# nasa/PROTEUS

Hardware: AMD Instinct MI355X
Metric: Mpixels/sec DSWx classify (3660^2 7-band HLS tiles) (higher is better)
Workload: dtype int16+f64

## Files before the change

### proteus_amd/build.py

```python
import contextlib
import fcntl
import hashlib
import os
import shutil
import subprocess
import sys

PKG = os.path.dirname(os.path.abspath(__file__))
ROOT = os.path.dirname(PKG)
CSRC = os.path.join(PKG, 'csrc')
LAB = os.path.join(ROOT, 'tools', 'lab', 'csrc')
SOURCES = [os.path.join(CSRC, n) for n in ('dswx_hip.hip', 'dswx_classify_lut.hip', 'dswx_cover.hip',
                                           'dswx_layers.hip', 'dswx_host_path.hip', 'dswx_batch.hip', 'dswx_writer.hip',
                                           'dswx_checksum.hip', 'dswx_compare.hip', 'dswx_histogram.hip', 'dswx_crosstab.hip',
                                           'dswx_stack.hip', 'dswx_grid.hip', 'dswx_label.hip', 'dswx_body_table.hip',
                                           'dswx_distance.hip', 'dswx_outline.hip', 'dswx_burn.hip', 'dswx_mosaic.hip', 'dswx_warp.hip',
                                           'dswx_resample.hip')]
HEADERS = [os.path.join(CSRC, n) for n in ('dswx_device.h', 'dswx_host.h', 'dswx_tables.h', 'dswx_vmm.h',
                                           'dswx_hist_bin.h', 'dswx_stack_rule.h', 'dswx_grid_rule.h',
                                           'dswx_label_rule.h', 'dswx_body_rule.h', 'dswx_distance_rule.h',
                                           'dswx_outline_rule.h', 'dswx_burn_rule.h', 'dswx_batch_select.h',
                                           'dswx_mesh_rule.h', 'dswx_resample_rule.h')]
LAB_SOURCES = [os.path.join(LAB, n) for n in ('dswx_lab.hip', 'dswx_probes.hip')]
LAB_HEADERS = [os.path.join(LAB, 'dswx_lab.h')]
INCLUDE = os.path.join(ROOT, 'include')
PUBLIC_HEADER = os.path.join(INCLUDE, 'dswx_hip.h')
LIB_DIR = os.path.join(PKG, '_lib')
LIB_PATH = os.path.join(LIB_DIR, 'libdswx_hip.so')
LAB_PATH = os.path.join(LIB_DIR, 'libdswx_lab.so')

HIPCC_FLAGS = ['--offload-arch=gfx950', '-O3', '-std=c++17', '-fPIC', '-shared',
               '-ffp-contract=off', '-Wall', '-Wno-unused-function']
HOT_KERNEL_SOURCES = [os.path.join(CSRC, n) for n in ('dswx_classify_lut.hip', 'dswx_tables.h', 'dswx_device.h')]


def find_hipcc():
    for cand in (shutil.which('hipcc'), '/opt/rocm/bin/hipcc'):
        if cand and os.path.exists(cand):
            return cand
    return None


def _digest(paths, extra=b''):
    h = hashlib.sha256(extra)
    for path in paths:
        h.update(os.path.basename(path).encode() + b'\0')
        with open(path, 'rb') as f:
            h.update(f.read())
        h.update(b'\0')
    return h.hexdigest()


def _stamp(lib):
    return lib + '.srchash'


def _stale(lib, deps, extra=b''):
    if not os.path.exists(lib) or not os.path.exists(_stamp(lib)):
        return True
    try:
        with open(_stamp(lib)) as f:
            return f.read().strip() != _digest(deps, extra)
    except OSError:
        return True


def _product_deps():
    return SOURCES + HEADERS + [PUBLIC_HEADER]


def _lab_deps():
    return LAB_SOURCES + LAB_HEADERS + HEADERS + [PUBLIC_HEADER]


def _flags_tag():
    return ' '.join(HIPCC_FLAGS).encode()


def is_stale():
    return _stale(LIB_PATH, _product_deps(), _flags_tag())


def _product_stamp():
    try:
        with open(_stamp(LIB_PATH)) as f:
            return f.read().strip().encode()
    except OSError:
        return b'missing'


def lab_is_stale():
    return _stale(LAB_PATH, _lab_deps(), _flags_tag() + _product_stamp())


def hot_kernel_hash():
    h = hashlib.sha256()
    for path in HOT_KERNEL_SOURCES:
        with open(path, 'rb') as f:
            h.update(f.read())
    return h.hexdigest()[:16]


def _run(cmd, verbose):
    if verbose:
        print(' '.join(cmd), file=sys.stderr)
    res = subprocess.run(cmd, capture_output=True, text=True)
    if res.returncode != 0:
        raise RuntimeError(f'{os.path.basename(cmd[0])} failed:\n' + res.stdout + res.stderr)


@contextlib.contextmanager
def _build_lock():
    os.makedirs(LIB_DIR, exist_ok=True)
    try:
        f = open(os.path.join(LIB_DIR, '.build.lock'), 'a')
    except OSError:
        yield
        return
    with f:
        fcntl.flock(f, fcntl.LOCK_EX)
        try:
            yield
        finally:
            fcntl.flock(f, fcntl.LOCK_UN)


def _write_stamp(lib, digest):
    tmp = f'{_stamp(lib)}.{os.getpid()}.tmp'
    with open(tmp, 'w') as f:
        f.write(digest + '\n')
    os.replace(tmp, _stamp(lib))


def _need_hipcc(lib):
    hipcc = find_hipcc()
    if hipcc is None:
        raise RuntimeError(f'hipcc not found and {os.path.relpath(lib, ROOT)} is '
                           + ('not the build of these sources (content digest differs)' if os.path.exists(lib) else 'missing')
                           + ' (need ROCm for the gfx950 build)')
    return hipcc


def build(force=False, verbose=False):
    if not force and not is_stale():
        return LIB_PATH
    with _build_lock():
        if not force and not is_stale():
            return LIB_PATH
        hipcc = _need_hipcc(LIB_PATH)
        tmp = f'{LIB_PATH}.{os.getpid()}.tmp'
        digest = _digest(_product_deps(), _flags_tag())
        _run([hipcc] + HIPCC_FLAGS + ['-I', INCLUDE, '-I', CSRC] + SOURCES + ['-o', tmp], verbose)
        if os.path.exists(_stamp(LIB_PATH)):
            os.remove(_stamp(LIB_PATH))
        os.replace(tmp, LIB_PATH)
        _write_stamp(LIB_PATH, digest)
    return LIB_PATH


def build_lab(force=False, verbose=False):
    build(force=False, verbose=verbose)
    if not force and not lab_is_stale():
        return LAB_PATH
    with _build_lock():
        if not force and not lab_is_stale():
            return LAB_PATH
        hipcc = _need_hipcc(LAB_PATH)
        tmp = f'{LAB_PATH}.{os.getpid()}.tmp'
        digest = _digest(_lab_deps(), _flags_tag() + _product_stamp())
        _run([hipcc] + HIPCC_FLAGS + ['-I', INCLUDE, '-I', CSRC, '-I', LAB] + LAB_SOURCES +
             ['-L', LIB_DIR, '-ldswx_hip', '-Wl,-rpath,$ORIGIN', '-o', tmp], verbose)
        if os.path.exists(_stamp(LAB_PATH)):
            os.remove(_stamp(LAB_PATH))
        os.replace(tmp, LAB_PATH)
        _write_stamp(LAB_PATH, digest)
# ... 74 lines not shown
```

### proteus_amd/csrc/dswx_host.h

```cpp
#pragma once

#include <hip/hip_runtime.h>
#include <cstddef>
#include <cstdint>
#include <cstring>
#include <mutex>
#include <string>

#include "dswx_device.h"
#include "dswx_mesh_rule.h"

struct dswx_workspace {
    void* p = nullptr;
    size_t bytes = 0;
};

struct dswx_ctx {
    int device = -1;
    hipStream_t stream = nullptr;
    enum { WS_STAGE, WS_PARTIALS, WS_FOLD, WS_COVER, WS_UNTILE, WS_COUNT };
    dswx_workspace ws[WS_COUNT];
    bool fold_clean = false;
    hipStream_t ws_last = nullptr;
    bool ws_used = false;
    hipEvent_t ws_event = nullptr;
    void* tables = nullptr;
    bool tables_valid = false;
    hipStream_t tables_stream = nullptr;
    alignas(8) unsigned char tables_params[1024] = {};
    hipStream_t h2d_stream = nullptr, d2h_stream = nullptr;
    hipEvent_t pipe_in[3] = {nullptr, nullptr, nullptr}, pipe_k[3] = {nullptr, nullptr, nullptr},
               pipe_out[3] = {nullptr, nullptr, nullptr};
    int64_t* pipe_counters = nullptr;
    size_t pipe_counters_cap = 0;
    int cover_kernel = 8;
    int host_pipeline = 2;
    int host_chunks = 8;
    int shadow_kernel = 0;
    int shadow_grid_pad = 1;
    std::string last_kernel;
    int tune_lut_wps = 0;
    int tune_lut_interleave = -1;
    int tune_wps = 6;
    int tune_fold = 1;
    int place_force_candidate = -1;
    int fused_variant = -1;
};

int dswx_ws_enter(dswx_ctx* ctx, hipStream_t s);
int dswx_ws_leave(dswx_ctx* ctx, hipStream_t s);

int dswx_fail(int code, const char* fmt, ...);
int dswx_make_dev_params(const dswx_params_t* p, DevParams* d);

#define HIP_TRY(expr)                                                                              \
    do {                                                                                           \
        hipError_t e__ = (expr);                                                                   \
        if (e__ != hipSuccess)                                                                     \
            return dswx_fail(DSWX_ERR_HIP, "%s failed: %s (%s:%d)", #expr, hipGetErrorString(e__), \
                             __FILE__, __LINE__);                                                  \
    } while (0)

std::mutex& dswx_va_mutex();
template <typename T>
static inline hipError_t dswx_locked_malloc(T** p, size_t n) {
    std::lock_guard<std::mutex> lock(dswx_va_mutex());
    return hipMalloc(reinterpret_cast<void**>(p), n);
}

static inline hipStream_t dswx_stream_of(const dswx_ctx* ctx, void* stream) { return stream ? (hipStream_t)stream : ctx->stream; }

struct dswx_call_scratch {
    hipStream_t s;
    void* p[4] = {nullptr, nullptr, nullptr, nullptr};
    int n = 0;
    bool queued = false;
    explicit dswx_call_scratch(hipStream_t stream) : s(stream) {}
    dswx_call_scratch(const dswx_call_scratch&) = delete;
    template <typename T>
    hipError_t take(T** out, size_t bytes) {
        if (n == 4) return hipErrorOutOfMemory;
        const hipError_t e = dswx_locked_malloc(out, bytes);
        if (e == hipSuccess) { p[n++] = *out; queued = true; }
        return e;
    }
    hipError_t sync() {
        const hipError_t e = hipStreamSynchronize(s);
        if (e == hipSuccess) queued = false;
        return e;
    }
    ~dswx_call_scratch() {
        if (queued) (void)hipStreamSynchronize(s);
        for (int i = 0; i < n; ++i) (void)hipFree(p[i]);
    }
};

static inline bool aligned_to(const void* p, size_t a) { return (reinterpret_cast<uintptr_t>(p) & (a - 1)) == 0; }

int dswx_ws_reserve(dswx_workspace& w, size_t need, hipStream_t s, bool whole_device = false);

struct dswx_plane_desc {
    const char* name;
    bool input;
    unsigned char bytes;
    signed char batch;
    unsigned short offset;
    signed char kind;
};
#define DSWX_BAND_(k) {"band[" #k "]", true, 2, DSWX_PLANE_BAND0 + k, offsetof(dswx_planes_in_t, band) + k * sizeof(void*), DSWX_CMP_I16}
#define DSWX_IN_(f, idx) {#f, true, 1, idx, offsetof(dswx_planes_in_t, f), DSWX_CMP_U8}
#define DSWX_OUT_(f, bytes, idx) \
    {#f, false, bytes, idx, offsetof(dswx_planes_out_t, f), bytes == 1 ? DSWX_CMP_U8 : bytes == 2 ? DSWX_CMP_U16 : DSWX_CMP_F64}
constexpr dswx_plane_desc DSWX_PLANES[] = {
    DSWX_BAND_(0), DSWX_BAND_(1), DSWX_BAND_(2), DSWX_BAND_(3), DSWX_BAND_(4), DSWX_BAND_(5),
    DSWX_IN_(fmask, DSWX_PLANE_FMASK), DSWX_IN_(land, DSWX_PLANE_LAND), DSWX_IN_(shad, DSWX_PLANE_SHAD),
    DSWX_IN_(ocean, DSWX_PLANE_OCEAN),
    DSWX_OUT_(diag, 2, DSWX_PLANE_DIAG), DSWX_OUT_(wtr1, 1, DSWX_PLANE_WTR1),
    DSWX_OUT_(wtr1_aerosol, 1, DSWX_PLANE_WTR1_AEROSOL), DSWX_OUT_(wtr2, 1, DSWX_PLANE_WTR2),
    DSWX_OUT_(wtr, 1, DSWX_PLANE_WTR), DSWX_OUT_(bwtr, 1, DSWX_PLANE_BWTR), DSWX_OUT_(conf, 1, DSWX_PLANE_CONF),
    DSWX_OUT_(cloud, 1, DSWX_PLANE_CLOUD), DSWX_OUT_(browse, 1, DSWX_PLANE_BROWSE),
    DSWX_OUT_(mndwi, 8, -1), DSWX_OUT_(ndvi, 8, -1), DSWX_OUT_(awesh, 8, -1),
};
#undef DSWX_BAND_
#undef DSWX_IN_
#undef DSWX_OUT_
constexpr int DSWX_N_PLANES = sizeof DSWX_PLANES / sizeof DSWX_PLANES[0];

constexpr bool dswx_planes_in_abi_order() {
    constexpr int n_in = sizeof(dswx_planes_in_t) / sizeof(void*);
    for (int i = 0; i < DSWX_N_PLANES; ++i) {
        const dswx_plane_desc& d = DSWX_PLANES[i];
        if (d.input != (i < n_in) || d.offset != (d.input ? i : i - n_in) * sizeof(void*)) return false;
        if (d.batch != (i < DSWX_PLANE_COUNTERS ? i : -1)) return false;
    }
    return true;
}
static_assert(sizeof(dswx_planes_in_t) + sizeof(dswx_planes_out_t) == DSWX_N_PLANES * sizeof(void*) &&
              dswx_planes_in_abi_order(), "DSWX_PLANES does not match dswx_planes_in_t / dswx_planes_out_t");

static inline char* dswx_plane_get(const dswx_plane_desc& d, const dswx_planes_in_t* in, const dswx_planes_out_t* out) {
    const char* s = d.input ? reinterpret_cast<const char*>(in) : reinterpret_cast<const char*>(out);
    char* p = nullptr;
    if (s) std::memcpy(&p, s + d.offset, sizeof p);
    return p;
}
static inline void dswx_plane_set(const dswx_plane_desc& d, dswx_planes_in_t* in, dswx_planes_out_t* out, const void* p) {
    char* s = d.input ? reinterpret_cast<char*>(in) : reinterpret_cast<char*>(out);
    if (s) std::memcpy(s + d.offset, &p, sizeof p);
}

constexpr int DSWX_FOLD_MAX_TILES = 16;

int dswx_lut_fold_group_log2(bool extras);
void dswx_lut_geometry(const dswx_ctx* ctx, long long groups, bool extras, int lead_max, int* threads, long long* gx);
int dswx_lut_launch(dswx_ctx* ctx, const KArgs& args, bool masks, dim3 grid, dim3 block, hipStream_t stream,
                    char* info, size_t info_len);

struct dswx_checksum_plane {
    const void* base;
    uint64_t tile_bytes;
    uint64_t stride_bytes;
};
int dswx_checksum_launch(dswx_ctx* ctx, const dswx_checksum_plane* planes, int n_planes, int64_t n_tiles, uint64_t* out,
                         hipStream_t s);

struct dswx_compare_pair {
    const void* a;
    const void* b;
    int kind;
    uint64_t n_elems;
    uint64_t a_stride_elems, b_stride_elems;
};
int dswx_compare_elem_bytes(int kind);
int dswx_compare_check_tol(double atol, double rtol);
int dswx_compare_launch(dswx_ctx* ctx, const dswx_compare_pair* pairs, int n_pairs, int64_t n_tiles, double atol, double rtol,
                        int equal_nan, dswx_compare_t* out, hipStream_t s);

struct dswx_histogram_plane {
    const void* base;
    int kind;
    int lo, shift;
    uint64_t n_elems;
    uint64_t stride_elems;
};
int dswx_histogram_elem_bytes(int kind);
int dswx_histogram_check_kind(int kind, int shift);
int dswx_histogram_launch(dswx_ctx* ctx, const dswx_histogram_plane* planes, int n_planes, int64_t n_tiles, uint64_t* out,
                          hipStream_t s);

struct dswx_crosstab_item {
    const void* a;
// ... 91 lines not shown
```

### proteus_amd/csrc/dswx_layers.hip

```cpp
#include <hip/hip_runtime.h>
#include <cmath>
#include <cstring>
#include <limits>

#include "dswx_host.h"

__global__ __launch_bounds__(256) void dswx_interpret_v1(const long long* __restrict__ diag,
                                                         uint8_t* __restrict__ out, long long n) {
    const long long i = (long long)blockIdx.x * 256 + threadIdx.x;
    if (i >= n) return;
    const long long d = diag[i];
    uint32_t cls = 255u;
    if (d >= 0 && d < 32) {
        const uint32_t k = (uint32_t)d;
        cls = ((CLS_B0 >> k) & 1u) | (((CLS_B1 >> k) & 1u) << 1) | (((CLS_B2 >> k) & 1u) << 2);
    }
    out[i] = (uint8_t)cls;
}

struct ShadowArgs {
    const float* dem;
    uint8_t* shadow;
    long long height, width, margin;
    long long out_stride;
    float spacing_x, neg_abs_spacing_y;
    double sun[3];
    double sin_az, cos_az;
    double inc_q_min, slope_arg_max;
    int by_first, by_step;
};

template <bool F32>
__device__ __forceinline__ bool shadow_px_exact(const ShadowArgs& a, float dx, float sx, float dy, float sy) {
    const float gx = dx * sx, gy = dy * sy;
    const float n0 = -gx / a.spacing_x;
    const float n1 = -gy / a.neg_abs_spacing_y;
    const float norm = sqrtf(n0 * n0 + n1 * n1 + 1.0f);
    bool low_inc, backslope;
    if (F32) {
        const float qf = (n0 * (float)a.sun[0] + n1 * (float)a.sun[1] + (float)a.sun[2]) / norm;
        const float tf = n0 * (float)a.sin_az + n1 * (float)a.cos_az;
        low_inc = (qf >= (float)a.inc_q_min) & (qf <= 1.0f);
        backslope = tf <= (float)a.slope_arg_max;
    } else {
        const double dot = (double)n0 * a.sun[0] + (double)n1 * a.sun[1] + a.sun[2];
        const double q = dot / (double)norm;
        const double t = (double)n0 * a.sin_az + (double)n1 * a.cos_az;
        low_inc = (q >= a.inc_q_min) & (q <= 1.0);
        backslope = t <= a.slope_arg_max;
    }
    return low_inc | !backslope;
}

template <bool F32>
__global__ __launch_bounds__(256) void dswx_shadow_v2(const ShadowArgs a) {
    const int W = (int)a.width, H = (int)a.height, margin = (int)a.margin;
    const int ow = W - 2 * margin, oh = H - 2 * margin;
    const int ox = blockIdx.x * 64 + (threadIdx.x & 63), oy = blockIdx.y * 4 + (threadIdx.x >> 6);
    if (ox >= ow || oy >= oh) return;
    const int x = ox + margin, y = oy + margin;
    const float* __restrict__ d = a.dem + (size_t)blockIdx.z * (size_t)H * (size_t)W;
    const int c = y * W + x;
    const bool x_in = (x > 0) & (x < W - 1), y_in = (y > 0) & (y < H - 1);
    const float dx = d[x < W - 1 ? c + 1 : c] - d[x > 0 ? c - 1 : c];
    const float dy = d[y < H - 1 ? c + W : c] - d[y > 0 ? c - W : c];
    const bool v = shadow_px_exact<F32>(a, dx, x_in ? 0.5f : 1.0f, dy, y_in ? 0.5f : 1.0f);
    a.shadow[(size_t)blockIdx.z * (size_t)a.out_stride + (size_t)(oy * ow + ox)] = v ? 1 : 0;
}

struct ShadowFilter {
    float inv_x, inv_y;
    float s0, s1, s2, sin_az, cos_az;
    float q_c, q_h_in, q_h_out;
    float t_c;
    float e_rel, e_abs;
    float et_rel;
    int t_tiny;
};

typedef float f32x2 __attribute__((ext_vector_type(2)));
typedef f32x2 __attribute__((aligned(4))) f32x2_u;
typedef uint32_t __attribute__((aligned(1))) u32_u;

template <bool F32, bool TINY>
__device__ __forceinline__ uint32_t shadow_quad(const ShadowArgs& a, const ShadowFilter& f, f32x2 c0, f32x2 c1, f32x2 c2,
                                                f32x2 c3, f32x2 u0, f32x2 u1, f32x2 b0, f32x2 b1) {
    const f32x2 dx[2] = {f32x2{c1.y, c2.x} - f32x2{c0.y, c1.x}, f32x2{c2.y, c3.x} - f32x2{c1.y, c2.x}};
    const f32x2 dy[2] = {b0 - u0, b1 - u1};
    uint32_t out = 0, unsure = 0;
#pragma unroll
    for (int p = 0; p < 2; ++p) {
        const f32x2 n0 = dx[p] * f.inv_x, n1 = dy[p] * f.inv_y;
        const f32x2 S = __builtin_elementwise_fma(n0, n0, __builtin_elementwise_fma(n1, n1, f32x2{1.0f, 1.0f}));
        const f32x2 dot = __builtin_elementwise_fma(n0, f32x2{f.s0, f.s0},
                                                    __builtin_elementwise_fma(n1, f32x2{f.s1, f.s1}, f32x2{f.s2, f.s2}));
        const f32x2 v = __builtin_elementwise_fma(n0, f32x2{f.sin_az, f.sin_az},
                                                  __builtin_elementwise_fma(n1, f32x2{f.cos_az, f.cos_az}, f32x2{-f.t_c, -f.t_c}));
        const f32x2 r = {__builtin_amdgcn_rsqf(S.x), __builtin_amdgcn_rsqf(S.y)};
        const f32x2 u = __builtin_elementwise_fma(dot, r, f32x2{-f.q_c, -f.q_c});
        f32x2 e = __builtin_elementwise_fma(S * r, f32x2{f.e_rel, f.e_rel}, f32x2{f.e_abs, f.e_abs});
        if (TINY) {
#pragma unroll
            for (int h = 0; h < 2; ++h)
                e[h] = f.et_rel * __builtin_fmaf(__builtin_fabsf(n0[h]), __builtin_fabsf(f.sin_az),
                                                 __builtin_fabsf(n1[h]) * __builtin_fabsf(f.cos_az)) +
                       __builtin_fminf((__builtin_fabsf(dx[p][h]) + __builtin_fabsf(dy[p][h])) * 0x1p100f, 0x1p-120f);
        }
#pragma unroll
        for (int h = 0; h < 2; ++h) {
            const bool sane = S[h] < 0x1p60f;
            const float au = __builtin_fabsf(u[h]), av = __builtin_fabsf(v[h]);
            const bool inc_yes = au <= f.q_h_in, inc_no = au > f.q_h_out;
            const bool back_known = av > e[h], back_no = back_known & (v[h] > 0.0f);
            const bool back_yes = TINY ? ((back_known & (v[h] < 0.0f)) | ((e[h] == 0.0f) & (v[h] <= 0.0f)))
                                           : (back_known & !(v[h] > 0.0f));
            const bool one = sane & (inc_yes | back_no);
            const bool zero = sane & inc_no & back_yes;
            const int k = 2 * p + h;
            out |= (one ? 1u : 0u) << (8 * k);
            unsure |= ((one | zero) ? 0u : 1u) << k;
        }
    }
    if (unsure) {
        const float cx[6] = {c0.y, c1.x, c1.y, c2.x, c2.y, c3.x};
        const float up[4] = {u0.x, u0.y, u1.x, u1.y}, dn[4] = {b0.x, b0.y, b1.x, b1.y};
#pragma unroll 1
        for (int k = 0; k < 4; ++k) {
            if (!((unsure >> k) & 1u)) continue;
            const bool v = shadow_px_exact<F32>(a, cx[k + 2] - cx[k], 0.5f, dn[k] - up[k], 0.5f);
            out = (out & ~(0xffu << (8 * k))) | ((v ? 1u : 0u) << (8 * k));
        }
    }
    return out;
}

constexpr int SHADOW_ROWS = 2, SHADOW_WAVES = 4;

template <bool F32, bool TINY>
__global__ __launch_bounds__(64 * SHADOW_WAVES) void dswx_shadow_v3(const ShadowArgs a, const ShadowFilter f) {
    const int W = (int)a.width, H = (int)a.height, margin = (int)a.margin;
    const int ow = W - 2 * margin, oh = H - 2 * margin;
    const int oq = blockIdx.x * 64 + (threadIdx.x & 63);
    const int oy0 = ((a.by_first + (int)blockIdx.y * a.by_step) * SHADOW_WAVES + (threadIdx.x >> 6)) * SHADOW_ROWS;
    if (4 * oq >= ow || oy0 >= oh) return;
    const int ox = 4 * oq + 4 <= ow ? 4 * oq : ow - 4;
    const float* __restrict__ col = a.dem + (size_t)blockIdx.z * (size_t)H * (size_t)W + (size_t)(ox + margin);
    uint8_t* __restrict__ dst = a.shadow + (size_t)blockIdx.z * (size_t)a.out_stride + (size_t)ox;
    struct Row { f32x2 v[4]; };
    auto load_row = [&](int y) {
        const float* r = col + (size_t)(y < H ? y : H - 1) * (size_t)W;
        return Row{{*reinterpret_cast<const f32x2_u*>(r - 2), *reinterpret_cast<const f32x2_u*>(r),
                    *reinterpret_cast<const f32x2_u*>(r + 2), *reinterpret_cast<const f32x2_u*>(r + 4)}};
    };
    const int y0 = oy0 + margin;
    Row up = load_row(y0 - 1), ce = load_row(y0), dn = load_row(y0 + 1), nx = SHADOW_ROWS > 1 ? load_row(y0 + 2) : dn;
#pragma unroll
    for (int i = 0; i < SHADOW_ROWS; ++i) {
        const Row nn = i + 3 <= SHADOW_ROWS ? load_row(y0 + i + 3) : nx;
        if (oy0 + i < oh) {
            const uint32_t out = shadow_quad<F32, TINY>(a, f, ce.v[0], ce.v[1], ce.v[2], ce.v[3], up.v[1], up.v[2], dn.v[1], dn.v[2]);
            __builtin_nontemporal_store(out, reinterpret_cast<u32_u*>(dst + (size_t)(oy0 + i) * (size_t)ow));
        }
        up = ce;
        ce = dn;
        dn = nx;
        nx = nn;
    }
}

struct LandArgs {
    const uint8_t* wc3;
    const uint8_t* cgls;
    uint8_t* land;
    long long height, width;
    long long out_stride;
    uint32_t forest_bits[8];
    int thr_tree, thr_low, thr_high, thr_water;
    int low_class, high_class;
};

__device__ __forceinline__ int land_class(const LandArgs& a, int water, int urban, int tree, bool is_forest) {
    if (!is_forest) tree = 0;
    int v = 255;
    if (tree >= a.thr_tree) v = 201;
    if (urban >= a.thr_low) v = a.low_class;
    if (urban >= a.thr_high) v = a.high_class;
    if (water >= a.thr_water) v = 200;
    return v;
}

constexpr int LAND_ROWS = 1;

__global__ __launch_bounds__(256) void dswx_landcover_v3(const LandArgs a) {
    __shared__ uint16_t s_code[256];
    __shared__ uint8_t s_forest[256];
    {
        const int v = threadIdx.x;
        s_code[v] = (uint16_t)((((v == 80) | (v == 90) | (v == 95)) ? 1 : 0) | (v == 50 ? 16 : 0) | (v == 10 ? 256 : 0));
        s_forest[v] = (uint8_t)((a.forest_bits[v >> 5] >> (v & 31)) & 1u);
    }
    __syncthreads();
    const unsigned quads_per_row = (unsigned)(a.width >> 2);
    const unsigned q = blockIdx.x * 256u + threadIdx.x;
    const unsigned yq = q / quads_per_row;
    const long long xq = q - yq * quads_per_row, y0 = yq;
    if (y0 >= a.height) return;
    const long long W3 = 3 * a.width, tile = blockIdx.z;
    const uint8_t* wc = a.wc3 + tile * 9 * a.height * a.width;
    uint32_t w[LAND_ROWS][3][3], cg[LAND_ROWS];
#pragma unroll
    for (int r = 0; r < LAND_ROWS; ++r) {
        const long long y = y0 + r < a.height ? y0 + r : a.height - 1;
#pragma unroll
        for (int i = 0; i < 3; ++i) {
            const uint32_t* row = reinterpret_cast<const uint32_t*>(wc + (3 * y + i) * W3 + 12 * xq);
#pragma unroll
            for (int k = 0; k < 3; ++k) w[r][i][k] = row[k];
        }
        cg[r] = __builtin_nontemporal_load(reinterpret_cast<const uint32_t*>(a.cgls + tile * a.height * a.width + y * a.width + 4 * xq));
    }
#pragma unroll
    for (int r = 0; r < LAND_ROWS; ++r) {
        if (y0 + r >= a.height) break;
        uint32_t cnt[4] = {0u, 0u, 0u, 0u};
#pragma unroll
        for (int i = 0; i < 3; ++i) {
#pragma unroll
            for (int j = 0; j < 12; ++j) cnt[j / 3] += s_code[(w[r][i][j >> 2] >> (8 * (j & 3))) & 0xffu];
        }
        uint32_t out = 0;
#pragma unroll
        for (int k = 0; k < 4; ++k)
            out |= (uint32_t)land_class(a, cnt[k] & 15u, (cnt[k] >> 4) & 15u, cnt[k] >> 8,
                                        s_forest[(cg[r] >> (8 * k)) & 0xffu] != 0) << (8 * k);
        __builtin_nontemporal_store(out, reinterpret_cast<uint32_t*>(a.land + tile * a.out_stride + (y0 + r) * a.width + 4 * xq));
    }
}

__global__ __launch_bounds__(256) void dswx_landcover_v1(const LandArgs a) {
    const long long x = (long long)blockIdx.x * 64 + (threadIdx.x & 63);
    const long long y = (long long)blockIdx.y * 4 + (threadIdx.x >> 6);
    if (x >= a.width || y >= a.height) return;
    int water = 0, urban = 0, tree = 0;
    const long long W3 = 3 * a.width;
    const long long tile = blockIdx.z;
#pragma unroll
    for (int i = 0; i < 3; ++i) {
        const uint8_t* row = a.wc3 + tile * 9 * a.height * a.width + (3 * y + i) * W3 + 3 * x;
#pragma unroll
        for (int j = 0; j < 3; ++j) {
            const int v = row[j];
            water += (v == 80) | (v == 90) | (v == 95);
            urban += v == 50;
            tree += v == 10;
        }
    }
    const long long o = tile * a.height * a.width + y * a.width + x;
    const int c = a.cgls[o];
    a.land[tile * a.out_stride + y * a.width + x] = (uint8_t)land_class(a, water, urban, tree, ((a.forest_bits[c >> 5] >> (c & 31)) & 1u) != 0);
}

__device__ __forceinline__ unsigned long long mix64(unsigned long long x) {
    x ^= x >> 30; x *= 0xBF58476D1CE4E5B9ull;
    x ^= x >> 27; x *= 0x94D049BB133111EBull;
    return x ^ (x >> 31);
}
__device__ __forceinline__ long long fieldu(unsigned long long h, int shift, int bits) {
    return (long long)((h >> shift) & ((1ull << bits) - 1ull));
}

__global__ __launch_bounds__(256) void dswx_synth_v1(dswx_planes_in_t in, unsigned long long seed,
                                                      long long tile0, long long n_pixels, int width,
                                                      long long tile_stride) {
    const long long px = (long long)blockIdx.x * 256 + threadIdx.x;
    if (px >= n_pixels) return;
    const long long t = blockIdx.y;
    const unsigned long long tile = (unsigned long long)(tile0 + t);
    const long long off = t * tile_stride + px;
    const unsigned long long K0 = 0x9E3779B97F4A7C15ull, K1 = 0xD1B54A32D192ED03ull;
    const unsigned long long h0 = mix64(seed * K0 + tile * K1 + (unsigned long long)px);
    const unsigned long long h1 = mix64(h0 + K0);
    const unsigned long long h2 = mix64(h1 + K0);
    const int cuts[5] = {14418, 26214, 42598, 55705, 64225};
    const int mean[5][6] = {{350, 450, 350, 250, 150, 100},
                            {500, 700, 600, 1300, 800, 500},
                            {300, 600, 400, 3500, 1800, 900},
                            {900, 1200, 1500, 2200, 2800, 2300},
                            {6000, 6200, 6400, 6600, 3000, 2500}};
    const int amps[5] = {300, 600, 600, 800, 2500};
    const int draw = (int)fieldu(h0, 0, 16);
    int stype = 0;
#pragma unroll
    for (int k = 0; k < 5; ++k) stype += draw >= cuts[k] ? 1 : 0;
    const bool is_fill = stype == 5;
    const int st = stype < 4 ? stype : 4;
    const long long amp = amps[st];
    const bool clip_evt = fieldu(h0, 16, 7) == 0;
    const int clip_band = (int)((fieldu(h0, 23, 3) * 6) >> 3);
    const long long clip_val = -fieldu(h0, 26, 8);
    const bool wrap_evt = fieldu(h0, 34, 10) == 0;
#pragma unroll
    for (int b = 0; b < 6; ++b) {
        const long long noise = fieldu(h1, 10 * b, 10);
        long long v = mean[st][b] + ((noise * 2 * amp) >> 10) - amp;
        if (wrap_evt && (b == 1 || b == 4)) v += 19000;
        if (clip_evt && clip_band == b) v = clip_val;
        if (is_fill) v = -9999;
        const_cast<int16_t*>(in.band[b])[off] = (int16_t)v;
    }
    const long long aerosol = fieldu(h2, 0, 2);
    const long long water = fieldu(h2, 2, 5) < 10, snow = fieldu(h2, 7, 5) < 2,
                    shadow = fieldu(h2, 12, 5) < 3, adjacent = fieldu(h2, 17, 5) < 3,
                    cloud = fieldu(h2, 22, 5) < 4, cirrus = fieldu(h2, 27, 5) < 1;
    long long fm = (aerosol << 6) | (water << 5) | (snow << 4) | (shadow << 3) | (adjacent << 2) |
                   (cloud << 1) | cirrus;
    if (is_fill) fm = 255;
    const_cast<uint8_t*>(in.fmask)[off] = (uint8_t)fm;
    if (in.land) {
        const int classes[8] = {200, 201, 21, 121, 50, 150, 99, 100};
        const int cls = classes[fieldu(h2, 40, 3)];
        const_cast<uint8_t*>(in.land)[off] = (uint8_t)(fieldu(h2, 32, 8) < 179 ? 255 : cls);
    }
    if (in.shad) const_cast<uint8_t*>(in.shad)[off] = (uint8_t)(fieldu(h2, 43, 5) >= 3 ? 1 : 0);
    if (in.ocean) {
        const unsigned long long row_band = (unsigned long long)(px / width) >> 5;
        const unsigned long long hb = mix64(seed * K1 + tile * K0 + row_band + 0x5851F42D4C957F2Dull);
        const_cast<uint8_t*>(in.ocean)[off] = (uint8_t)(fieldu(hb, 0, 8) >= 13 ? 1 : 0);
    }
}

extern "C" {

#define ENTRY_TRY(entry, expr)                                                                                      \
    do {                                                                                                            \
        if (hipError_t e__ = (expr)) return dswx_fail(DSWX_ERR_HIP, entry ": %s", hipGetErrorString(e__));          \
    } while (0)

int dswx_interpret_layer_host(dswx_ctx_t* ctx, const int64_t* diag_decimal, int64_t n, uint8_t* out) {
    if (!ctx || (n > 0 && (!diag_decimal || !out))) return dswx_fail(DSWX_ERR_ARG, "NULL argument");
    if (n < 0) return dswx_fail(DSWX_ERR_ARG, "negative size");
    if (n == 0) return DSWX_OK;
    HIP_TRY(hipSetDevice(ctx->device));
    dswx_call_scratch scratch(ctx->stream);
    long long* d_in = nullptr; uint8_t* d_out = nullptr;
    ENTRY_TRY("dswx_interpret_layer_host", scratch.take(&d_in, (size_t)n * 8));
    ENTRY_TRY("dswx_interpret_layer_host", scratch.take(&d_out, (size_t)n));
    ENTRY_TRY("dswx_interpret_layer_host", hipMemcpyAsync(d_in, diag_decimal, (size_t)n * 8, hipMemcpyHostToDevice, scratch.s));
    hipLaunchKernelGGL(dswx_interpret_v1, dim3((unsigned)((n + 255) / 256)), dim3(256), 0, scratch.s, d_in, d_out, (long long)n);
    ENTRY_TRY("dswx_interpret_layer_host", hipGetLastError());
    ENTRY_TRY("dswx_interpret_layer_host", hipMemcpyAsync(out, d_out, (size_t)n, hipMemcpyDeviceToHost, scratch.s));
    ENTRY_TRY("dswx_interpret_layer_host", scratch.sync());
    return DSWX_OK;
}

static int64_t ord_of(double d) {
    int64_t i;
    std::memcpy(&i, &d, 8);
    return i >= 0 ? i : -(i & 0x7fffffffffffffffLL);
}
static double dbl_of(int64_t k) {
    int64_t i = k >= 0 ? k : (int64_t)(0x8000000000000000ULL | (uint64_t)(-k));
    double d;
    std::memcpy(&d, &i, 8);
    return d;
}
static const double kRad2Deg = 180.0 / 3.141592653589793238462643383279502884;

int dswx_shadow_thresholds(double min_slope_angle, double max_sun_local_inc_angle, double* slope_arg_max,
                           double* inc_q_min) {
    if (!slope_arg_max || !inc_q_min) return dswx_fail(DSWX_ERR_ARG, "NULL argument");
    if (std::isnan(min_slope_angle) || std::isnan(max_sun_local_inc_angle))
        return dswx_fail(DSWX_ERR_ARG, "shadow angle threshold is NaN");
    auto inc_ok = [&](double q) { return std::acos(q) * kRad2Deg <= max_sun_local_inc_angle; };
    if (!inc_ok(1.0)) *inc_q_min = 2.0;
    else if (inc_ok(-1.0)) *inc_q_min = -1.0;
    else {
        int64_t lo = ord_of(-1.0), hi = ord_of(1.0);
        while ((uint64_t)hi - (uint64_t)lo > 1) {
            const int64_t mid = lo + (int64_t)(((uint64_t)hi - (uint64_t)lo) / 2);
            if (inc_ok(dbl_of(mid))) hi = mid; else lo = mid;
        }
        *inc_q_min = dbl_of(hi);
    }
    auto slope_ok = [&](double t) { return std::atan(t) * kRad2Deg <= min_slope_angle; };
    const double inf = std::numeric_limits<double>::infinity();
    if (slope_ok(inf)) *slope_arg_max = inf;
    else if (!slope_ok(-inf)) *slope_arg_max = -inf;
    else {
        int64_t lo = ord_of(-inf), hi = ord_of(inf);
// ... 68 lines not shown
        f->t_c = t_max > 0 ? std::numeric_limits<float>::infinity() : -std::numeric_limits<float>::infinity();
        f->e_abs = 0.0f;
    } else {
        f->t_c = (float)t_max;
        f->e_abs = f->t_tiny ? 0.0f : float_up(std::fabs((double)f->t_c - t_max) + std::fabs(t_max) * 0x1p-20 + 1e-40);
    }
}

static int shadow_launch(dswx_ctx_t* ctx, const ShadowArgs& req, int64_t n_tiles, bool f32, hipStream_t s) {
    if (n_tiles == 0) return DSWX_OK;
    HIP_TRY(hipSetDevice(ctx->device));
    ShadowArgs a = req;
    const long long margin = a.margin, ow = a.width - 2 * margin, oh = a.height - 2 * margin;
    const bool quads = margin >= 2 && ow >= 4 && aligned_to(a.dem, 4) && ctx->shadow_kernel != 2;
    if (quads) {
        ShadowFilter f;
        shadow_filter(a, f32, &f);
        const long long pad = ctx->shadow_grid_pad > 0 ? ctx->shadow_grid_pad : 1;
        const long long gx = (((ow + 3) / 4 + 63) / 64 + pad - 1) / pad * pad;
        const unsigned block_rows = (unsigned)((oh + SHADOW_WAVES * SHADOW_ROWS - 1) / (SHADOW_WAVES * SHADOW_ROWS));
        const dim3 block(64 * SHADOW_WAVES);
        const int passes = ctx->shadow_kernel == 3 ? 2 : 1;
        for (int pass = 0; pass < passes; ++pass) {
            a.by_first = pass; a.by_step = passes;
            const unsigned gy = (block_rows - (unsigned)pass + (unsigned)passes - 1) / (unsigned)passes;
            if (gy == 0) continue;
            const dim3 grid((unsigned)gx, gy, (unsigned)n_tiles);
            if (f32 && f.t_tiny) hipLaunchKernelGGL((dswx_shadow_v3<true, true>), grid, block, 0, s, a, f);
            else if (f32) hipLaunchKernelGGL((dswx_shadow_v3<true, false>), grid, block, 0, s, a, f);
            else if (f.t_tiny) hipLaunchKernelGGL((dswx_shadow_v3<false, true>), grid, block, 0, s, a, f);
            else hipLaunchKernelGGL((dswx_shadow_v3<false, false>), grid, block, 0, s, a, f);
        }
    } else {
        dim3 grid((unsigned)((ow + 63) / 64), (unsigned)((oh + 3) / 4), (unsigned)n_tiles), block(256);
        if (f32) hipLaunchKernelGGL(dswx_shadow_v2<true>, grid, block, 0, s, a);
        else hipLaunchKernelGGL(dswx_shadow_v2<false>, grid, block, 0, s, a);
    }
    HIP_TRY(hipGetLastError());
    return DSWX_OK;
}

static int shadow_host_run(dswx_ctx_t* ctx, ShadowArgs a, bool f32) {
    const float* dem = a.dem; uint8_t* shadow = a.shadow;
    HIP_TRY(hipSetDevice(ctx->device));
    const size_t in_bytes = (size_t)a.height * (size_t)a.width * 4;
    const size_t out_px = (size_t)(a.height - 2 * a.margin) * (size_t)(a.width - 2 * a.margin);
    dswx_call_scratch scratch(ctx->stream);
    float* d_dem = nullptr; uint8_t* d_out = nullptr;
    ENTRY_TRY("dswx_shadow_layer_host", scratch.take(&d_dem, in_bytes));
    ENTRY_TRY("dswx_shadow_layer_host", scratch.take(&d_out, out_px));
    ENTRY_TRY("dswx_shadow_layer_host", hipMemcpyAsync(d_dem, dem, in_bytes, hipMemcpyHostToDevice, scratch.s));
    a.dem = d_dem; a.shadow = d_out;
    if (int rc = shadow_launch(ctx, a, 1, f32, scratch.s)) return rc;
    ENTRY_TRY("dswx_shadow_layer_host", hipMemcpyAsync(shadow, d_out, out_px, hipMemcpyDeviceToHost, scratch.s));
    ENTRY_TRY("dswx_shadow_layer_host", scratch.sync());
    return DSWX_OK;
}

int dswx_shadow_layer_device_q(dswx_ctx_t* ctx, const float* dem, int64_t n_tiles, int64_t height, int64_t width,
                               int64_t margin, const double sun_vector[3], double sin_azimuth,
                               double cos_azimuth, double slope_arg_max, double inc_q_min,
                               double pixel_spacing_x, double pixel_spacing_y, uint8_t* shadow, void* stream) {
    ShadowArgs a;
    if (int rc = shadow_check(&a, ctx, dem, n_tiles, height, width, margin, sun_vector, sin_azimuth, cos_azimuth, slope_arg_max,
                              inc_q_min, pixel_spacing_x, pixel_spacing_y, shadow, 0)) return rc;
    return shadow_launch(ctx, a, n_tiles, false, dswx_stream_of(ctx, stream));
}

int dswx_shadow_layer_device_q32(dswx_ctx_t* ctx, const float* dem, int64_t n_tiles, int64_t height, int64_t width,
                                 int64_t margin, const double sun_vector[3], double sin_azimuth,
                                 double cos_azimuth, float slope_arg_max, float inc_q_min,
                                 double pixel_spacing_x, double pixel_spacing_y, uint8_t* shadow, void* stream) {
    ShadowArgs a;
    if (int rc = shadow_check(&a, ctx, dem, n_tiles, height, width, margin, sun_vector, sin_azimuth, cos_azimuth,
                              (double)slope_arg_max, (double)inc_q_min, pixel_spacing_x, pixel_spacing_y, shadow, 0)) return rc;
    return shadow_launch(ctx, a, n_tiles, true, dswx_stream_of(ctx, stream));
}

int dswx_shadow_layer_device(dswx_ctx_t* ctx, const float* dem, int64_t n_tiles, int64_t height, int64_t width,
                             int64_t margin, const double sun_vector[3], double sin_azimuth,
                             double cos_azimuth, double min_slope_angle, double max_sun_local_inc_angle,
                             double pixel_spacing_x, double pixel_spacing_y, uint8_t* shadow, void* stream) {
    double slope_arg_max, inc_q_min;
    if (int rc = dswx_shadow_thresholds(min_slope_angle, max_sun_local_inc_angle, &slope_arg_max, &inc_q_min)) return rc;
    ShadowArgs a;
    if (int rc = shadow_check(&a, ctx, dem, n_tiles, height, width, margin, sun_vector, sin_azimuth, cos_azimuth, slope_arg_max,
                              inc_q_min, pixel_spacing_x, pixel_spacing_y, shadow, 0)) return rc;
    return shadow_launch(ctx, a, n_tiles, false, dswx_stream_of(ctx, stream));
}

int dswx_shadow_layer_batch(dswx_ctx_t* ctx, const float* dem, int64_t n_tiles, int64_t height, int64_t width,
                            int64_t margin, const double sun_vector[3], double sin_azimuth, double cos_azimuth,
                            double slope_arg_max, double inc_q_min, int32_t float32_arithmetic, double pixel_spacing_x,
                            double pixel_spacing_y, uint8_t* shadow, int64_t shadow_tile_stride, void* stream) {
    ShadowArgs a;
    if (int rc = shadow_check(&a, ctx, dem, n_tiles, height, width, margin, sun_vector, sin_azimuth, cos_azimuth, slope_arg_max,
                              inc_q_min, pixel_spacing_x, pixel_spacing_y, shadow, shadow_tile_stride)) return rc;
    return shadow_launch(ctx, a, n_tiles, float32_arithmetic != 0, dswx_stream_of(ctx, stream));
}

int dswx_shadow_layer_host_q(dswx_ctx_t* ctx, const float* dem, int64_t height, int64_t width, int64_t margin,
                             const double sun_vector[3], double sin_azimuth, double cos_azimuth,
                             double slope_arg_max, double inc_q_min, double pixel_spacing_x,
                             double pixel_spacing_y, uint8_t* shadow) {
    ShadowArgs a;
    if (int rc = shadow_check(&a, ctx, dem, 1, height, width, margin, sun_vector, sin_azimuth, cos_azimuth, slope_arg_max,
                              inc_q_min, pixel_spacing_x, pixel_spacing_y, shadow, 0)) return rc;
    return shadow_host_run(ctx, a, false);
}

int dswx_shadow_layer_host_q32(dswx_ctx_t* ctx, const float* dem, int64_t height, int64_t width, int64_t margin,
                               const double sun_vector[3], double sin_azimuth, double cos_azimuth,
                               float slope_arg_max, float inc_q_min, double pixel_spacing_x,
                               double pixel_spacing_y, uint8_t* shadow) {
    ShadowArgs a;
    if (int rc = shadow_check(&a, ctx, dem, 1, height, width, margin, sun_vector, sin_azimuth, cos_azimuth,
                              (double)slope_arg_max, (double)inc_q_min, pixel_spacing_x, pixel_spacing_y, shadow, 0)) return rc;
    return shadow_host_run(ctx, a, true);
}

int dswx_shadow_layer_host(dswx_ctx_t* ctx, const float* dem, int64_t height, int64_t width, int64_t margin,
                           const double sun_vector[3], double sin_azimuth, double cos_azimuth,
                           double min_slope_angle, double max_sun_local_inc_angle, double pixel_spacing_x,
                           double pixel_spacing_y, uint8_t* shadow) {
    double slope_arg_max, inc_q_min;
    if (int rc = dswx_shadow_thresholds(min_slope_angle, max_sun_local_inc_angle, &slope_arg_max, &inc_q_min)) return rc;
    ShadowArgs a;
    if (int rc = shadow_check(&a, ctx, dem, 1, height, width, margin, sun_vector, sin_azimuth, cos_azimuth, slope_arg_max,
                              inc_q_min, pixel_spacing_x, pixel_spacing_y, shadow, 0)) return rc;
    return shadow_host_run(ctx, a, false);
}

static int land_check(LandArgs* a, dswx_ctx_t* ctx, const uint8_t* worldcover_up3, const uint8_t* copernicus, int64_t n_tiles,
                      int64_t height, int64_t width, const int32_t* forest_classes, int32_t n_forest_classes,
                      const int32_t thresholds[4], int32_t year_offset, uint8_t* land, int64_t land_tile_stride) {
    if (!ctx || !worldcover_up3 || !copernicus || !land) return dswx_fail(DSWX_ERR_ARG, "NULL argument");
    if (land_tile_stride != 0 && land_tile_stride < height * width)
        return dswx_fail(DSWX_ERR_ARG, "land_tile_stride smaller than the raster");
    if (n_tiles < 0 || n_tiles > 65535) return dswx_fail(DSWX_ERR_ARG, "n_tiles out of range");
    if (!thresholds) return dswx_fail(DSWX_ERR_ARG, "NULL argument");
    if (height < 0 || width < 0 || n_forest_classes < 0 || (n_forest_classes > 0 && !forest_classes))
        return dswx_fail(DSWX_ERR_ARG, "bad size");
    std::memset(a, 0, sizeof *a);
    for (int i = 0; i < n_forest_classes; ++i) {
        const int c = forest_classes[i];
        if (c >= 0 && c <= 255) a->forest_bits[c >> 5] |= 1u << (c & 31);
    }
    a->thr_tree = thresholds[0]; a->thr_low = thresholds[1]; a->thr_high = thresholds[2]; a->thr_water = thresholds[3];
    a->low_class = (int)(uint8_t)(0u + (uint32_t)year_offset);
    a->high_class = (int)(uint8_t)(100u + (uint32_t)year_offset);
    a->height = height; a->width = width;
    a->wc3 = worldcover_up3; a->cgls = copernicus; a->land = land;
    a->out_stride = land_tile_stride ? land_tile_stride : height * width;
    return DSWX_OK;
}

static int land_launch(dswx_ctx_t* ctx, const LandArgs& a, int64_t n_tiles, hipStream_t s) {
    const long long height = a.height, width = a.width;
    if (n_tiles == 0 || height == 0 || width == 0) return DSWX_OK;
    HIP_TRY(hipSetDevice(ctx->device));
    const bool quad = width % 4 == 0 && aligned_to(a.wc3, 4) && aligned_to(a.cgls, 4) && aligned_to(a.land, 4) &&
                      a.out_stride % 4 == 0;
    if (quad) {
        static_assert(LAND_ROWS == 1, "the flat quad numbering assumes one row per thread");
        const long long quads = (width / 4) * height;
        if (quads > 0xffffffffLL - 256) return dswx_fail(DSWX_ERR_ARG, "raster too large for one launch");
        dim3 grid((unsigned)((quads + 255) / 256), 1, (unsigned)n_tiles), block(256);
        hipLaunchKernelGGL(dswx_landcover_v3, grid, block, 0, s, a);
    } else {
        dim3 grid((unsigned)((width + 63) / 64), (unsigned)((height + 3) / 4), (unsigned)n_tiles), block(256);
        if (grid.y > 65535) return dswx_fail(DSWX_ERR_ARG, "raster too tall for one launch");
        hipLaunchKernelGGL(dswx_landcover_v1, grid, block, 0, s, a);
    }
    HIP_TRY(hipGetLastError());
    return DSWX_OK;
}

int dswx_landcover_mask_device(dswx_ctx_t* ctx, const uint8_t* worldcover_up3, const uint8_t* copernicus,
                               int64_t n_tiles, int64_t height, int64_t width, const int32_t* forest_classes,
                               int32_t n_forest_classes, const int32_t thresholds[4], int32_t year_offset,
                               uint8_t* land, void* stream) {
    LandArgs a;
    if (int rc = land_check(&a, ctx, worldcover_up3, copernicus, n_tiles, height, width, forest_classes, n_forest_classes,
                            thresholds, year_offset, land, 0)) return rc;
    return land_launch(ctx, a, n_tiles, dswx_stream_of(ctx, stream));
}

int dswx_landcover_mask_batch(dswx_ctx_t* ctx, const uint8_t* worldcover_up3, const uint8_t* copernicus,
                              int64_t n_tiles, int64_t height, int64_t width, const int32_t* forest_classes,
                              int32_t n_forest_classes, const int32_t thresholds[4], int32_t year_offset,
                              uint8_t* land, int64_t land_tile_stride, void* stream) {
    LandArgs a;
    if (int rc = land_check(&a, ctx, worldcover_up3, copernicus, n_tiles, height, width, forest_classes, n_forest_classes,
                            thresholds, year_offset, land, land_tile_stride)) return rc;
    return land_launch(ctx, a, n_tiles, dswx_stream_of(ctx, stream));
}

int dswx_landcover_mask_host(dswx_ctx_t* ctx, const uint8_t* worldcover_up3, const uint8_t* copernicus,
                             int64_t height, int64_t width, const int32_t* forest_classes,
                             int32_t n_forest_classes, const int32_t thresholds[4], int32_t year_offset,
                             uint8_t* land) {
    LandArgs a;
    if (int rc = land_check(&a, ctx, worldcover_up3, copernicus, 1, height, width, forest_classes, n_forest_classes,
                            thresholds, year_offset, land, 0)) return rc;
    if (height == 0 || width == 0) return DSWX_OK;
    HIP_TRY(hipSetDevice(ctx->device));
    const size_t n = (size_t)height * (size_t)width;
    dswx_call_scratch scratch(ctx->stream);
    uint8_t* d_wc = nullptr; uint8_t* d_cg = nullptr; uint8_t* d_out = nullptr;
    ENTRY_TRY("dswx_landcover_mask_host", scratch.take(&d_wc, 9 * n));
    ENTRY_TRY("dswx_landcover_mask_host", scratch.take(&d_cg, n));
    ENTRY_TRY("dswx_landcover_mask_host", scratch.take(&d_out, n));
    ENTRY_TRY("dswx_landcover_mask_host", hipMemcpyAsync(d_wc, worldcover_up3, 9 * n, hipMemcpyHostToDevice, scratch.s));
    ENTRY_TRY("dswx_landcover_mask_host", hipMemcpyAsync(d_cg, copernicus, n, hipMemcpyHostToDevice, scratch.s));
    a.wc3 = d_wc; a.cgls = d_cg; a.land = d_out;
    if (int rc = land_launch(ctx, a, 1, scratch.s)) return rc;
    ENTRY_TRY("dswx_landcover_mask_host", hipMemcpyAsync(land, d_out, n, hipMemcpyDeviceToHost, scratch.s));
    ENTRY_TRY("dswx_landcover_mask_host", scratch.sync());
    return DSWX_OK;
}

static int synth_impl(dswx_ctx_t* ctx, uint64_t seed, int64_t tile0, int64_t n_tiles, int64_t height,
                      int64_t width, int64_t tile_stride, const dswx_planes_in_t* in, void* stream) {
    if (!ctx || !in) return dswx_fail(DSWX_ERR_ARG, "NULL argument");
    if (n_tiles < 0 || height < 0 || width < 0 || tile0 < 0) return dswx_fail(DSWX_ERR_ARG, "negative size");
    for (int k = 0; k < 6; ++k)
        if (!in->band[k]) return dswx_fail(DSWX_ERR_ARG, "band[%d] is NULL", k);
    if (!in->fmask) return dswx_fail(DSWX_ERR_ARG, "fmask is NULL");
    const int64_t P = height * width;
    if (tile_stride == 0) tile_stride = P;
    if (tile_stride < P) return dswx_fail(DSWX_ERR_ARG, "tile_stride smaller than the tile");
    if (n_tiles == 0 || P == 0) return DSWX_OK;
    HIP_TRY(hipSetDevice(ctx->device));
    hipStream_t s = dswx_stream_of(ctx, stream);
    const int64_t max_y = 65535;
    for (int64_t t0 = 0; t0 < n_tiles; t0 += max_y) {
        const int64_t nt = (n_tiles - t0 < max_y) ? n_tiles - t0 : max_y;
        dswx_planes_in_t b = *in;
        const int64_t shift = t0 * tile_stride;
        for (int k = 0; k < 6; ++k) b.band[k] += shift;
        b.fmask += shift;
        if (b.land) b.land += shift;
        if (b.shad) b.shad += shift;
        if (b.ocean) b.ocean += shift;
        dim3 grid((unsigned)((P + 255) / 256), (unsigned)nt), block(256);
        hipLaunchKernelGGL(dswx_synth_v1, grid, block, 0, s, b, (unsigned long long)seed,
                           (long long)(tile0 + t0), (long long)P, (int)width, (long long)tile_stride);
        HIP_TRY(hipGetLastError());
    }
    return DSWX_OK;
}

int dswx_synth_fill(dswx_ctx_t* ctx, uint64_t seed, int64_t tile0, int64_t n_tiles, int64_t height,
                    int64_t width, const dswx_planes_in_t* in, void* stream) {
    return synth_impl(ctx, seed, tile0, n_tiles, height, width, 0, in, stream);
}

int dswx_synth_batch(dswx_ctx_t* ctx, uint64_t seed, int64_t tile0, const dswx_batch_geom_t* geom,
                     const dswx_planes_in_t* in, void* stream) {
    if (!geom) return dswx_fail(DSWX_ERR_ARG, "geom is NULL");
    return synth_impl(ctx, seed, tile0, geom->n_tiles, geom->height, geom->width, geom->tile_stride, in, stream);
}

}
```

Baseline: 310,000.

## Add landcover v4 kernel with packed SWAR counts and threshold-word classification

Adds a new landcover kernel that packs water/urban/tree counts into bit fields of one 32-bit word. Thresholds are pre-biased so a single add and a multiply-gather yield a 4-bit pass mask, which indexes a precomputed 16-entry class table. It also replaces 64-bit index math with a magic-number divide and 32-bit offsets, fills the shared LUT via inverse ballot, and hoists the global loads above the barrier. The new kernel is the default on the quad path. It adds template variants and a lever selector, and the 32-bit offsets are guarded by a size check.

After: 307,800. About the same (-0.7%).

```diff
diff --git a/proteus_amd/build.py b/proteus_amd/build.py
--- a/proteus_amd/build.py
+++ b/proteus_amd/build.py
@@ -20,7 +20,7 @@
                                            'dswx_hist_bin.h', 'dswx_stack_rule.h', 'dswx_grid_rule.h',
                                            'dswx_label_rule.h', 'dswx_body_rule.h', 'dswx_distance_rule.h',
                                            'dswx_outline_rule.h', 'dswx_burn_rule.h', 'dswx_batch_select.h',
-                                           'dswx_mesh_rule.h', 'dswx_resample_rule.h')]
+                                           'dswx_mesh_rule.h', 'dswx_resample_rule.h', 'dswx_land_rule.h')]
 LAB_SOURCES = [os.path.join(LAB, n) for n in ('dswx_lab.hip', 'dswx_probes.hip')]
 LAB_HEADERS = [os.path.join(LAB, 'dswx_lab.h')]
 INCLUDE = os.path.join(ROOT, 'include')
diff --git a/proteus_amd/csrc/dswx_host.h b/proteus_amd/csrc/dswx_host.h
--- a/proteus_amd/csrc/dswx_host.h
+++ b/proteus_amd/csrc/dswx_host.h
@@ -37,6 +37,7 @@
     int host_pipeline = 2;
     int host_chunks = 8;
     int shadow_kernel = 0;
+    int land_kernel = 0;
     int shadow_grid_pad = 1;
     std::string last_kernel;
     int tune_lut_wps = 0;
diff --git a/proteus_amd/csrc/dswx_land_rule.h b/proteus_amd/csrc/dswx_land_rule.h
--- /dev/null
+++ b/proteus_amd/csrc/dswx_land_rule.h
@@ -0,0 +1,65 @@
+#pragma once
+#include <cstdint>
+
+namespace {
+
+__host__ __device__ __forceinline__ int land_clamp_thr(int thr) { return thr < 0 ? 0 : thr > 10 ? 10 : thr; }
+
+enum : uint32_t {
+    LAND_F_WATER = 0, LAND_F_LOW = 6, LAND_F_HIGH = 12, LAND_F_TREE = 18,
+    LAND_ONE_WATER = 1u << LAND_F_WATER, LAND_ONE_URBAN = (1u << LAND_F_LOW) | (1u << LAND_F_HIGH), LAND_ONE_TREE = 1u << LAND_F_TREE,
+    LAND_PASS_BITS = (32u << LAND_F_WATER) | (32u << LAND_F_LOW) | (32u << LAND_F_HIGH) | (32u << LAND_F_TREE),
+    LAND_GATHER = (1u << 23) | (1u << 18) | (1u << 13) | (1u << 8),
+    LAND_P_WATER = 1, LAND_P_LOW = 2, LAND_P_HIGH = 4, LAND_P_TREE = 8,
+};
+
+__host__ __device__ __forceinline__ uint32_t land_code_word(unsigned wc_byte) {
+    return (((wc_byte == 80) | (wc_byte == 90) | (wc_byte == 95)) ? LAND_ONE_WATER : 0u) | (wc_byte == 50 ? LAND_ONE_URBAN : 0u) |
+           (wc_byte == 10 ? LAND_ONE_TREE : 0u);
+}
+
+__host__ __device__ __forceinline__ uint32_t land_threshold_word(const int thr[4], bool is_forest) {
+    const uint32_t tree = (uint32_t)land_clamp_thr(thr[0]);
+    return ((32u - (uint32_t)land_clamp_thr(thr[3])) << LAND_F_WATER) | ((32u - (uint32_t)land_clamp_thr(thr[1])) << LAND_F_LOW) |
+           ((32u - (uint32_t)land_clamp_thr(thr[2])) << LAND_F_HIGH) | ((is_forest ? 32u - tree : tree == 0 ? 32u : 0u) << LAND_F_TREE);
+}
+
+__host__ __device__ __forceinline__ uint32_t land_passed(uint32_t sum) { return ((sum & LAND_PASS_BITS) * LAND_GATHER) >> 28; }
+
+__host__ __device__ __forceinline__ void land_class_table(uint8_t table[16], int low_class, int high_class) {
+    for (unsigned p = 0; p < 16; ++p) {
+        int v = 255;
+        if (p & LAND_P_TREE) v = 201;
+        if (p & LAND_P_LOW) v = low_class;
+        if (p & LAND_P_HIGH) v = high_class;
+        if (p & LAND_P_WATER) v = 200;
+        table[p] = (uint8_t)v;
+    }
+}
+
+struct LandDiv {
+    uint32_t mul, sh1, sh2;
+};
+
+inline LandDiv land_div_make(uint32_t d) {
+    if (d <= 1) return LandDiv{0u, 0u, 0u};
+    uint32_t s = 0;
+    while ((1ull << s) < d) ++s;
+    const unsigned __int128 M = ((unsigned __int128)1 << (32 + s)) / d + 1;
+    return LandDiv{(uint32_t)(uint64_t)M, 1u, s - 1};
+}
+
+__host__ __device__ __forceinline__ uint32_t land_div(uint32_t q, const LandDiv& m) {
+#if defined(__HIP_DEVICE_COMPILE__)
+    const uint32_t t = __umulhi(q, m.mul);
+#else
+    const uint32_t t = (uint32_t)(((uint64_t)q * m.mul) >> 32);
+#endif
+    return (t + ((q - t) >> m.sh1)) >> m.sh2;
+}
+
+__host__ __device__ __forceinline__ bool land_offsets_fit32(long long height, long long width) {
+    return height > 0 && width > 0 && height <= 0xffffffffLL / 9 / width;
+}
+
+}
diff --git a/proteus_amd/csrc/dswx_layers.hip b/proteus_amd/csrc/dswx_layers.hip
--- a/proteus_amd/csrc/dswx_layers.hip
+++ b/proteus_amd/csrc/dswx_layers.hip
@@ -1,9 +1,11 @@
 #include <hip/hip_runtime.h>
 #include <cmath>
+#include <cstdio>
 #include <cstring>
 #include <limits>
 
 #include "dswx_host.h"
+#include "dswx_land_rule.h"
 
 __global__ __launch_bounds__(256) void dswx_interpret_v1(const long long* __restrict__ diag,
                                                          uint8_t* __restrict__ out, long long n) {
@@ -177,6 +179,11 @@
     uint32_t forest_bits[8];
     int thr_tree, thr_low, thr_high, thr_water;
     int low_class, high_class;
+    uint32_t thr_word[2];
+    uint32_t class_table[4];
+    uint32_t quads_per_row;
+    LandDiv row_of_quad;
+    uint32_t n_quads;
 };
 
 __device__ __forceinline__ int land_class(const LandArgs& a, int water, int urban, int tree, bool is_forest) {
@@ -235,6 +242,88 @@
                                         s_forest[(cg[r] >> (8 * k)) & 0xffu] != 0) << (8 * k);
         __builtin_nontemporal_store(out, reinterpret_cast<uint32_t*>(a.land + tile * a.out_stride + (y0 + r) * a.width + 4 * xq));
     }
+}
+
+constexpr int LAND_V4_DEFAULT = 15;
+
+template <int LEVERS>
+__global__ __launch_bounds__(256) void dswx_landcover_v4(const LandArgs a) {
+    constexpr bool SCALAR_FILL = LEVERS & 1, FAST_INDEX = LEVERS & 2, HOIST = LEVERS & 4, NT_STORE = LEVERS & 8;
+    __shared__ uint32_t s_code[256];
+    __shared__ uint32_t s_thr[256];
+    __shared__ uint32_t s_class[4];
+    const unsigned tid = threadIdx.x;
+    const unsigned q = blockIdx.x * 256u + tid;
+    const bool live = q < a.n_quads;
+    const unsigned qc = live ? q : a.n_quads - 1;
+    const unsigned yq = FAST_INDEX ? land_div(qc, a.row_of_quad) : qc / a.quads_per_row;
+    const unsigned row_first = yq * a.quads_per_row;
+    const long long tile = blockIdx.z;
+    const uint8_t* wc = a.wc3 + tile * 9 * a.height * a.width;
+    const uint8_t* cgls = a.cgls + tile * a.height * a.width;
+    uint32_t w[3][3], cg;
+    auto load = [&]() {
+        if (FAST_INDEX) {
+            const unsigned W3 = 3u * (unsigned)a.width, off = 12u * (qc + 2u * row_first);
+#pragma unroll
+            for (int i = 0; i < 3; ++i) {
+                const uint32_t* row = reinterpret_cast<const uint32_t*>(wc + (off + i * W3));
+#pragma unroll
+                for (int k = 0; k < 3; ++k) w[i][k] = row[k];
+            }
+            cg = __builtin_nontemporal_load(reinterpret_cast<const uint32_t*>(cgls + 4u * qc));
+        } else {
+            const long long W3 = 3 * a.width;
+#pragma unroll
+            for (int i = 0; i < 3; ++i) {
+                const uint32_t* row = reinterpret_cast<const uint32_t*>(wc + (3ll * yq + i) * W3 + 12ll * (qc - row_first));
+#pragma unroll
+                for (int k = 0; k < 3; ++k) w[i][k] = row[k];
+            }
+            cg = __builtin_nontemporal_load(reinterpret_cast<const uint32_t*>(cgls + 4ll * qc));
+        }
+    };
+    if (HOIST) load();
+    if (SCALAR_FILL) {
+        const unsigned wave = __builtin_amdgcn_readfirstlane(tid >> 6);
+        const unsigned long long tree = wave == 0 ? 1ull << 10 : 0ull, urban = wave == 0 ? 1ull << 50 : 0ull;
+        const unsigned long long water = wave == 1 ? (1ull << (80 - 64)) | (1ull << (90 - 64)) | (1ull << (95 - 64)) : 0ull;
+        const unsigned long long forest = ((unsigned long long)a.forest_bits[2 * wave + 1] << 32) | a.forest_bits[2 * wave];
+        s_code[tid] = (__builtin_amdgcn_inverse_ballot_w64(water) ? LAND_ONE_WATER : 0u) |
+                      (__builtin_amdgcn_inverse_ballot_w64(urban) ? LAND_ONE_URBAN : 0u) |
+                      (__builtin_amdgcn_inverse_ballot_w64(tree) ? LAND_ONE_TREE : 0u);
+        s_thr[tid] = __builtin_amdgcn_inverse_ballot_w64(forest) ? a.thr_word[0] : a.thr_word[1];
+    } else {
+        s_code[tid] = land_code_word(tid);
+        s_thr[tid] = a.thr_word[(a.forest_bits[tid >> 5] >> (tid & 31)) & 1u ? 0 : 1];
+    }
+    if (tid == 0) {
+#pragma unroll
+        for (int k = 0; k < 4; ++k) s_class[k] = a.class_table[k];
+    }
+    __syncthreads();
+    if (!HOIST) load();
+    uint32_t out = 0;
+#pragma unroll
+    for (int k = 0; k < 4; ++k) {
+        uint32_t sum = s_thr[(cg >> (8 * k)) & 0xffu];
+#pragma unroll
+        for (int i = 0; i < 3; ++i) {
+#pragma unroll
+            for (int j = 3 * k; j < 3 * k + 3; ++j) sum += s_code[(w[i][j >> 2] >> (8 * (j & 3))) & 0xffu];
+        }
+        out |= (uint32_t)reinterpret_cast<const uint8_t*>(s_class)[land_passed(sum)] << (8 * k);
+    }
+    if (!live) return;
+    uint8_t* land = a.land + tile * a.out_stride;
+    uint32_t* dst = FAST_INDEX ? reinterpret_cast<uint32_t*>(land + 4u * q) : reinterpret_cast<uint32_t*>(land + 4ll * q);
+    if (NT_STORE) __builtin_nontemporal_store(out, dst);
+    else *dst = out;
+}
+
+template <int LEVERS>
+static void land_v4_launch(const LandArgs& a, dim3 grid, hipStream_t s) {
+    hipLaunchKernelGGL(dswx_landcover_v4<LEVERS>, grid, dim3(256), 0, s, a);
 }
 
 __global__ __launch_bounds__(256) void dswx_landcover_v1(const LandArgs a) {
@@ -609,13 +698,26 @@
     a->height = height; a->width = width;
     a->wc3 = worldcover_up3; a->cgls = copernicus; a->land = land;
     a->out_stride = land_tile_stride ? land_tile_stride : height * width;
+    const int thr[4] = {a->thr_tree, a->thr_low, a->thr_high, a->thr_water};
+    a->thr_word[0] = land_threshold_word(thr, true);
+    a->thr_word[1] = land_threshold_word(thr, false);
+    uint8_t classes[16];
+    land_class_table(classes, a->low_class, a->high_class);
+    std::memcpy(a->class_table, classes, sizeof classes);
+    a->quads_per_row = (uint32_t)(width / 4 < 0xffffffffLL ? width / 4 : 0xffffffffLL);
+    a->row_of_quad = land_div_make(a->quads_per_row);
+    a->n_quads = 0;
     return DSWX_OK;
 }
 
 static int land_launch(dswx_ctx_t* ctx, const LandArgs& a, int64_t n_tiles, hipStream_t s) {
     const long long height = a.height, width = a.width;
-    if (n_tiles == 0 || height == 0 || width == 0) return DSWX_OK;
+    if (n_tiles == 0 || height == 0 || width == 0) {
+        ctx->last_kernel = "none (empty input)";
+        return DSWX_OK;
+    }
     HIP_TRY(hipSetDevice(ctx->device));
+    char info[96];
     const bool quad = width % 4 == 0 && aligned_to(a.wc3, 4) && aligned_to(a.cgls, 4) && aligned_to(a.land, 4) &&
                       a.out_stride % 4 == 0;
     if (quad) {
@@ -623,13 +725,37 @@
         const long long quads = (width / 4) * height;
         if (quads > 0xffffffffLL - 256) return dswx_fail(DSWX_ERR_ARG, "raster too large for one launch");
         dim3 grid((unsigned)((quads + 255) / 256), 1, (unsigned)n_tiles), block(256);
-        hipLaunchKernelGGL(dswx_landcover_v3, grid, block, 0, s, a);
+        int levers = ctx->land_kernel >= 16 ? ctx->land_kernel - 16 : LAND_V4_DEFAULT;
+        if (!land_offsets_fit32(height, width)) {
+            if (ctx->land_kernel >= 16 && (levers & 2)) return dswx_fail(DSWX_ERR_ARG, "land_kernel: raster too large for 32-bit offsets");
+            levers &= ~2;
+        }
+        if (ctx->land_kernel == 3) {
+            hipLaunchKernelGGL(dswx_landcover_v3, grid, block, 0, s, a);
+            std::snprintf(info, sizeof info, "dswx_landcover_v3 grid=(%u,1,%u)", grid.x, grid.z);
+        } else {
+            LandArgs b = a;
+            b.n_quads = (uint32_t)quads;
+            switch (levers) {
+                case 0: land_v4_launch<0>(b, grid, s); break;
+                case 1: land_v4_launch<1>(b, grid, s); break;
+                case 3: land_v4_launch<3>(b, grid, s); break;
+                case 7: land_v4_launch<7>(b, grid, s); break;
+                case 11: land_v4_launch<11>(b, grid, s); break;
+                case 13: land_v4_launch<13>(b, grid, s); break;
+                case 15: land_v4_launch<15>(b, grid, s); break;
+                default: return dswx_fail(DSWX_ERR_ARG, "land_kernel: no dswx_landcover_v4<%d>", levers);
+            }
+            std::snprintf(info, sizeof info, "dswx_landcover_v4<%d> grid=(%u,1,%u)", levers, grid.x, grid.z);
+        }
     } else {
         dim3 grid((unsigned)((width + 63) / 64), (unsigned)((height + 3) / 4), (unsigned)n_tiles), block(256);
         if (grid.y > 65535) return dswx_fail(DSWX_ERR_ARG, "raster too tall for one launch");
         hipLaunchKernelGGL(dswx_landcover_v1, grid, block, 0, s, a);
+        std::snprintf(info, sizeof info, "dswx_landcover_v1 grid=(%u,%u,%u)", grid.x, grid.y, grid.z);
     }
     HIP_TRY(hipGetLastError());
+    ctx->last_kernel = info;
     return DSWX_OK;
 }
 
```
